# jaak-s/libfastsparse

Measured on AMD Instinct MI355X. Metric: fp64 CSR SpMV effective GB/s (% HBM3E peak), higher is better.
Workload: dtype f64

## Files before the change

libfastsparse_amd/csrc/fs_kernels_twopass.hip:

```cpp
#include <stdlib.h>

#include "fs_kernel_util.h"

namespace fs {


template <int U, bool NTLD, bool NTST, int BC>
__device__ __forceinline__ void expand_share(double *__restrict__ xband, int ncol, int B, const unsigned *__restrict__ band_ptr,
                                             const uint16_t *__restrict__ lcol, const unsigned *__restrict__ gdst,
                                             const double *__restrict__ x, int xs, double *__restrict__ prod, unsigned g0,
                                             unsigned g1)
{
  const int t = threadIdx.x;
  if (g0 >= g1) return;
  int b;
  {
    int lo = 0, hi = B - 1;
    while (lo < hi) {
      const int mid = lo + ((hi - lo + 1) >> 1);
      if (band_ptr[mid] <= g0) lo = mid; else hi = mid - 1;
    }
    b = lo;
  }
  for (unsigned g = g0; g < g1; ++b) {
    const unsigned gb = band_ptr[b + 1] < g1 ? band_ptr[b + 1] : g1;
    if (gb <= g) continue;
    const int c0 = b * BC;
    const int w = (ncol - c0 < BC) ? ncol - c0 : BC;
    __syncthreads();
    {
      double r[BC / kBinBlock];
#pragma unroll
      for (int j = 0; j < BC / kBinBlock; ++j) {
        const int i = j * kBinBlock + t;
        r[j] = __builtin_nontemporal_load(x + (int64_t)(c0 + (i < w ? i : w - 1)) * xs);
      }
#pragma unroll
      for (int j = 0; j < BC / kBinBlock; ++j) {
        const int i = j * kBinBlock + t;
        xband[i] = (i < w) ? r[j] : 0.0;
      }
      if (t < 8) xband[BC + t] = 0.0;
    }
    __syncthreads();
    const int64_t e0 = (int64_t)g * kBinGroup, e1 = (int64_t)gb * kBinGroup;
    constexpr int64_t kRound = 2 * U * kBinBlock;
    int64_t o = e0 + 2 * t;
    for (; o - 2 * t + kRound <= e1; o += kRound) {
      unsigned a[U], d[U];
#pragma unroll
      for (int k = 0; k < U; ++k) {
        const int64_t e = o + (int64_t)k * 2 * kBinBlock;
        a[k] = stream_load<NTLD>((const unsigned *)(lcol + e));
        d[k] = stream_load<NTLD>(gdst + (e >> kBinGroupLog));
      }
      __builtin_amdgcn_sched_barrier(0);
#pragma unroll
      for (int k = 0; k < U; ++k) {
        const int64_t e = o + (int64_t)k * 2 * kBinBlock;
        const v2d p = {xband[a[k] & 0xffffu], xband[a[k] >> 16]};
        stream_store<NTST>(p, (v2d *)(prod + (int64_t)d[k] * kBinGroup + (e & (kBinGroup - 1))));
      }
    }
    for (; o < e1; o += 2 * kBinBlock) {
      const unsigned a = stream_load<NTLD>((const unsigned *)(lcol + o));
      const unsigned d = stream_load<NTLD>(gdst + (o >> kBinGroupLog));
      const v2d p = {xband[a & 0xffffu], xband[a >> 16]};
      stream_store<NTST>(p, (v2d *)(prod + (int64_t)d * kBinGroup + (o & (kBinGroup - 1))));
    }
    g = gb;
  }
}

template <int U, bool NTLD, bool NTST, int BC = kBinCols>
__global__ __launch_bounds__(kBinBlock) void spmv_expand_kernel(
    int ncol, int B, const unsigned *__restrict__ band_ptr, const uint16_t *__restrict__ lcol,
    const unsigned *__restrict__ gdst, const double *__restrict__ x, int xs, double *__restrict__ prod, unsigned gbeg,
    unsigned gend)
{
  __shared__ double xband[BC + 8];
  const uint64_t groups = gend - gbeg;
  const unsigned g0 = gbeg + (unsigned)(groups * blockIdx.x / gridDim.x), g1 = gbeg + (unsigned)(groups * (blockIdx.x + 1) / gridDim.x);
  expand_share<U, NTLD, NTST, BC>(xband, ncol, B, band_ptr, lcol, gdst, x, xs, prod, g0, g1);
}

static_assert(kBinGroupLog == 4, "the one-byte row ids (row_ids, line_ids, rows8_decode_kernel) decode groups of 16 entries: two lanes of 8, eight lanes of 2, four words of 4");
template <bool NTLD, bool L8>
__device__ __forceinline__ v4u row_ids_load(const uint16_t *__restrict__ lrow, const uint8_t *__restrict__ lrow8,
                                            const uint16_t *__restrict__ gbase, int64_t e)
{
  if (!L8) return stream_load<NTLD>((const v4u *)(lrow + e));
  typedef unsigned v2u __attribute__((ext_vector_type(2)));
  const v2u d = stream_load<NTLD>((const v2u *)(lrow8 + e));
  return v4u{d.x, d.y, (unsigned)gbase[e >> kBinGroupLog], (unsigned)(e >> 3) & 1u};
}

template <bool L8>
__device__ __forceinline__ v4u row_ids(v4u raw)
{
  if (!L8) return raw;
  const unsigned dx = raw.x, dy = raw.y;
  const unsigned s0 = dx & 0xffu, s1 = s0 + ((dx >> 8) & 0xffu), s2 = s1 + ((dx >> 16) & 0xffu), s3 = s2 + (dx >> 24);
  const unsigned s4 = s3 + (dy & 0xffu), s5 = s4 + ((dy >> 8) & 0xffu), s6 = s5 + ((dy >> 16) & 0xffu), s7 = s6 + (dy >> 24);
  const unsigned below = (unsigned)__builtin_amdgcn_update_dpp(0, (int)s7, 0x111 , 0xf, 0xf, false);
  const unsigned off = raw.z + (raw.w ? below : 0u);
  return v4u{(off + s0) | ((off + s1) << 16), (off + s2) | ((off + s3) << 16), (off + s4) | ((off + s5) << 16), (off + s6) | ((off + s7) << 16)};
}

template <bool L8>
__device__ __forceinline__ unsigned line_ids_load(const uint16_t *__restrict__ lrow, const uint8_t *__restrict__ lrow8,
                                                  const uint16_t *__restrict__ gbase, int64_t e)
{
  if (!L8) return *(const unsigned *)(lrow + e);
  return (unsigned)*(const uint16_t *)(lrow8 + e) | ((unsigned)gbase[e >> kBinGroupLog] << 16);
}

template <bool L8>
__device__ __forceinline__ unsigned line_ids(unsigned raw)
{
  if (!L8) return raw;
  const unsigned d0 = raw & 0xffu, own = d0 + ((raw >> 8) & 0xffu), l = threadIdx.x & 7u;
  unsigned s = own, u;
  u = (unsigned)__builtin_amdgcn_update_dpp(0, (int)s, 0x111 , 0xf, 0xf, false); s += l >= 1 ? u : 0u;
  u = (unsigned)__builtin_amdgcn_update_dpp(0, (int)s, 0x112 , 0xf, 0xf, false); s += l >= 2 ? u : 0u;
  u = (unsigned)__builtin_amdgcn_update_dpp(0, (int)s, 0x114 , 0xf, 0xf, false); s += l >= 4 ? u : 0u;
  const unsigned off = (raw >> 16) + s - own;
  return (off + d0) | ((off + own) << 16);
}

template <bool VALUED, bool NTLD, bool L8 = false>
__device__ __forceinline__ void reduce_panel(double *__restrict__ ytile, int panel, const unsigned *__restrict__ bin_ptr,
                                             const int *__restrict__ panel_row, const uint16_t *__restrict__ lrow,
                                             const double *__restrict__ vals, const double *__restrict__ prod, double *__restrict__ y,
                                             int ys, const uint8_t *__restrict__ lrow8 = nullptr,
                                             const uint16_t *__restrict__ gbase = nullptr)
{
  const int t = threadIdx.x;
  const int r0 = panel_row[panel], nr = panel_row[panel + 1] - r0;
  for (int i = t; i < nr; i += kBinBlock) ytile[i] = 0.0;
  __syncthreads();
  const int64_t e0 = (int64_t)bin_ptr[panel] * kBinGroup, e1 = (int64_t)bin_ptr[panel + 1] * kBinGroup;
#define FS_ADD(idx, val) __hip_atomic_fetch_add(&ytile[idx], val, __ATOMIC_RELAXED, __HIP_MEMORY_SCOPE_WORKGROUP)
#define FS_ADD2(A, P) FS_ADD((A) & 0xffffu, (P).x); FS_ADD((A) >> 16, (P).y);
  constexpr int64_t kStep = 8 * kBinBlock, kRound = 2 * kStep;
  const int wave0 = (t >> 6) * 512, lane0 = wave0 + 2 * (t & 63);
  int64_t eb = e0;
  for (; eb + kRound <= e1; eb += kRound) {
    const int64_t e = eb + lane0;
    unsigned a[2][4];
    v2d p[2][4], v[2][4];
#pragma unroll
    for (int k = 0; k < 2; ++k)
#pragma unroll
      for (int j = 0; j < 4; ++j) {
        const int64_t ek = e + k * kStep + 128 * j;
        a[k][j] = line_ids_load<L8>(lrow, lrow8, gbase, ek);
        p[k][j] = stream_load<NTLD>((const v2d *)(prod + ek));
        if (VALUED) v[k][j] = stream_load<NTLD>((const v2d *)(vals + ek));
      }
    __builtin_amdgcn_sched_barrier(0);
#pragma unroll
    for (int k = 0; k < 2; ++k)
#pragma unroll
      for (int j = 0; j < 4; ++j) {
        const unsigned r = line_ids<L8>(a[k][j]);
        if (VALUED) { p[k][j].x *= v[k][j].x; p[k][j].y *= v[k][j].y; }
        FS_ADD2(r, p[k][j])
      }
  }
  for (; eb + wave0 < e1; eb += kStep) {
    const int64_t e = eb + lane0;
    unsigned a[4];
    v2d p[4], v[4];
#pragma unroll
    for (int j = 0; j < 4; ++j) {
      const int64_t ej = e + 128 * j, ec = ej < e1 ? ej : e1 - 2;
      a[j] = line_ids_load<L8>(lrow, lrow8, gbase, ec);
      p[j] = stream_load<NTLD>((const v2d *)(prod + ec));
      if (VALUED) v[j] = stream_load<NTLD>((const v2d *)(vals + ec));
    }
#pragma unroll
    for (int j = 0; j < 4; ++j) {
      const unsigned r = line_ids<L8>(a[j]);
      if (VALUED) { p[j].x *= v[j].x; p[j].y *= v[j].y; }
      if (e + 128 * j < e1) { FS_ADD2(r, p[j]) }
    }
  }
#undef FS_ADD2
#undef FS_ADD
  __syncthreads();
  for (int i = t; i < nr; i += kBinBlock) y[(int64_t)(r0 + i) * ys] = ytile[i];
}

template <bool VALUED, bool NTLD, int RM = kBinRowsMax, bool L8 = false>
__global__ __launch_bounds__(kBinBlock) void spmv_reduce_kernel(
    const unsigned *__restrict__ bin_ptr, const int *__restrict__ panel_row, const uint16_t *__restrict__ lrow,
    const double *__restrict__ vals, const double *__restrict__ prod, double *__restrict__ y, int ys, int pbase,
    const uint8_t *__restrict__ lrow8 = nullptr, const uint16_t *__restrict__ gbase = nullptr)
{
  __shared__ double ytile[RM];
  reduce_panel<VALUED, NTLD, L8>(ytile, pbase + blockIdx.x, bin_ptr, panel_row, lrow, vals, prod, y, ys, lrow8, gbase);
}

#ifndef FS_ORDERED_DEPTH
#define FS_ORDERED_DEPTH 16
#endif
#ifndef FS_ORDERED_DEPTH_VALUED
#define FS_ORDERED_DEPTH_VALUED 10
#endif
template <bool VALUED, bool NTLD, int RM, int DEPTH, bool L8 = false>
__global__ __launch_bounds__(64) void spmv_reduce_ordered_kernel(
    const unsigned *__restrict__ bin_ptr, const int *__restrict__ panel_row, const uint16_t *__restrict__ lrow,
    const double *__restrict__ vals, const double *__restrict__ prod, double *__restrict__ y, int ys, int pbase,
    const uint8_t *__restrict__ lrow8 = nullptr, const uint16_t *__restrict__ gbase = nullptr)
{
  __shared__ __attribute__((aligned(16))) double ytile[RM];
  const int t = threadIdx.x;
  const int panel = pbase + blockIdx.x;
  const int r0 = panel_row[panel], nr = panel_row[panel + 1] - r0;
  for (int i = 2 * t; i < nr; i += 128) *reinterpret_cast<v2d *>(&ytile[i]) = v2d{0.0, 0.0};
  const int64_t e0 = (int64_t)bin_ptr[panel] * kBinGroup, e1 = (int64_t)bin_ptr[panel + 1] * kBinGroup;
#define FS_ADD(idx, val) __hip_atomic_fetch_add(&ytile[idx], val, __ATOMIC_RELAXED, __HIP_MEMORY_SCOPE_WORKGROUP)
#define FS_ADD8(A, P)                                                  \
  FS_ADD(A.x & 0xffffu, P[0].x); FS_ADD(A.x >> 16, P[0].y);            \
  FS_ADD(A.y & 0xffffu, P[1].x); FS_ADD(A.y >> 16, P[1].y);            \
  FS_ADD(A.z & 0xffffu, P[2].x); FS_ADD(A.z >> 16, P[2].y);            \
  FS_ADD(A.w & 0xffffu, P[3].x); FS_ADD(A.w >> 16, P[3].y);
  constexpr int64_t kStep = 8 * 64;
  v4u a[DEPTH];
  v2d p[DEPTH][4], v[VALUED ? DEPTH : 1][4];
  auto fetch = [&](int k, int64_t e) {
    const int64_t ec = (e + 8 <= e1) ? e : (e1 - e0 >= 8 ? e1 - 8 : e0);
    a[k] = row_ids_load<NTLD, L8>(lrow, lrow8, gbase, ec);
#pragma unroll
    for (int j = 0; j < 4; ++j) {
      p[k][j] = stream_load<NTLD>((const v2d *)(prod + ec + 2 * j));
      if (VALUED) v[k][j] = stream_load<NTLD>((const v2d *)(vals + ec + 2 * j));
    }
  };
  if (e1 > e0) {
    int64_t e = e0 + 8 * t;
#pragma unroll
    for (int k = 0; k < DEPTH; ++k) fetch(k, e + (int64_t)k * kStep);
    for (; e - 8 * t < e1; e += (int64_t)DEPTH * kStep) {
#pragma unroll
      for (int k = 0; k < DEPTH; ++k) {
        const int64_t ek = e + (int64_t)k * kStep;
        const v4u ak = row_ids<L8>(a[k]);
        v2d pk[4] = {p[k][0], p[k][1], p[k][2], p[k][3]};
        if (VALUED) {
#pragma unroll
          for (int j = 0; j < 4; ++j) { pk[j].x *= v[k][j].x; pk[j].y *= v[k][j].y; }
        }
        fetch(k, ek + (int64_t)DEPTH * kStep);
        if (ek + 8 <= e1) { FS_ADD8(ak, pk) }
      }
    }
  }
#undef FS_ADD8
#undef FS_ADD
  __syncthreads();
  for (int i = t; i < nr; i += 64) y[(int64_t)(r0 + i) * ys] = ytile[i];
}

template <bool VALUED, int BC, int NACC, bool ORDERED>
__global__ __launch_bounds__(kBinBlock) void spmv_longrows_kernel(
    int ncol, int B, int nlong, const int64_t *__restrict__ band_ptr, const unsigned *__restrict__ seg_ptr,
    const uint16_t *__restrict__ lcol, const uint16_t *__restrict__ lrow, const double *__restrict__ vals,
    const double *__restrict__ x, int xs, double *__restrict__ ylong, double *__restrict__ ypart)
{
  __shared__ double xband[BC + 8];
  __shared__ double acc[NACC];
  const int t = threadIdx.x, lane = t & 63, wave = t >> 6;
  for (int i = t; i < nlong; i += kBinBlock) acc[i] = 0.0;
  const int64_t pairs = band_ptr[B] >> 1;
  const int64_t e_beg = 2 * (pairs * blockIdx.x / gridDim.x), e_end = 2 * (pairs * (blockIdx.x + 1) / gridDim.x);
  if (e_beg < e_end) {
    int b;
    {
      int lo = 0, hi = B - 1;
      while (lo < hi) {
        const int mid = lo + ((hi - lo + 1) >> 1);
        if (band_ptr[mid] <= e_beg) lo = mid; else hi = mid - 1;
      }
      b = lo;
    }
    double rn[BC / kBinBlock];
    int have = -1;
    auto request = [&](int bb) {
      const int cb = bb * BC;
      const int wb = (ncol - cb < BC) ? ncol - cb : BC;
#pragma unroll
      for (int j = 0; j < BC / kBinBlock; ++j) {
        const int i = j * kBinBlock + t;
        rn[j] = __builtin_nontemporal_load(x + (int64_t)(cb + (i < wb ? i : wb - 1)) * xs);
      }
      have = bb;
    };
    auto wave_step = [&](int64_t o, bool live, int64_t oc) {
      const unsigned a = *reinterpret_cast<const unsigned *>(lcol + oc);
      const unsigned rr = *reinterpret_cast<const unsigned *>(lrow + oc);
      v2d p = {xband[a & 0xffffu], xband[a >> 16]};
      if (VALUED) { const v2d v = *reinterpret_cast<const v2d *>(vals + oc); p.x *= v.x; p.y *= v.y; }
      unsigned key = 0xffffffffu;
      double sum = 0.0;
      if (live) {
        const unsigned r0 = rr & 0xffffu, r1 = rr >> 16;
        if (r0 == r1) { key = r0; sum = p.x + p.y; }
        else { __hip_atomic_fetch_add(&acc[r0], p.x, __ATOMIC_RELAXED, __HIP_MEMORY_SCOPE_WORKGROUP); key = r1; sum = p.y; }
      }
#pragma unroll
      for (int d = 1; d < 64; d <<= 1) {
        const unsigned ku = __shfl_up(key, d);
        const double su = __shfl_up(sum, d);
        if (lane >= d && ku == key) sum += su;
      }
      const unsigned kn = __shfl_down(key, 1);
      if (live && (lane == 63 || kn != key))
        __hip_atomic_fetch_add(&acc[key], sum, __ATOMIC_RELAXED, __HIP_MEMORY_SCOPE_WORKGROUP);
      (void)o;
    };
    for (int64_t e = e_beg; e < e_end; ++b) {
      const int64_t eb = band_ptr[b + 1] < e_end ? band_ptr[b + 1] : e_end;
      if (eb <= e) continue;
      const int c0 = b * BC;
      const int w = (ncol - c0 < BC) ? ncol - c0 : BC;
      if (have != b) request(b);
      __syncthreads();
#pragma unroll
      for (int j = 0; j < BC / kBinBlock; ++j) {
        const int i = j * kBinBlock + t;
        xband[i] = (i < w) ? rn[j] : 0.0;
      }
      if (t < 8) xband[BC + t] = 0.0;
      __syncthreads();
      if (b + 1 < B && eb < e_end) request(b + 1);
      if (ORDERED) {
        const int64_t s0 = band_ptr[b] + seg_ptr[b * (kLongOwners + 1) + wave], s1 = band_ptr[b] + seg_ptr[b * (kLongOwners + 1) + wave + 1];
        const int64_t lo = s0 > e ? s0 : e, hi = s1 < eb ? s1 : eb;
        for (int64_t o0 = lo; o0 < hi; o0 += 128) {
          const int64_t o = o0 + 2 * lane;
          const bool live = o < hi;
          wave_step(o, live, live ? o : lo);
        }
      } else {
        for (int64_t o0 = e; o0 < eb; o0 += 2 * kBinBlock) {
          const int64_t o = o0 + 2 * t;
          const bool live = o < eb;
          wave_step(o, live, live ? o : e);
        }
      }
      e = eb;
    }
  }
  __syncthreads();
  if (ORDERED) {
    double *__restrict__ mine = ypart + (int64_t)blockIdx.x * nlong;
    for (int i = t; i < nlong; i += kBinBlock) mine[i] = acc[i];
  } else {
    for (int i = t; i < nlong; i += kBinBlock) {
      const double v = acc[i];
      if (v != 0.0) unsafeAtomicAdd(ylong + i, v);
    }
  }
}

__global__ __launch_bounds__(kBlock) void longrows_combine_kernel(int nlong, int nwg, const double *__restrict__ ypart, double *__restrict__ ylong)
{
  const int i = blockIdx.x * kBlock + threadIdx.x;
  if (i >= nlong) return;
  double acc = 0.0;
  for (int w = 0; w < nwg; ++w) acc += ypart[(int64_t)w * nlong + i];
  ylong[i] = acc;
}

__global__ __launch_bounds__(kBlock) void longrows_scatter_kernel(int nlong, const int *__restrict__ row, const double *__restrict__ ylong,
                                                                 double *__restrict__ y, int ys, int row0, int row1)
{
  const int i = blockIdx.x * kBlock + threadIdx.x;
  if (i >= nlong) return;
  const int r = row[i];
  if (r >= row0 && r < row1) y[(int64_t)r * ys] = 0.0 + ylong[i];
}

static int launch_longrows(const DeviceCsr &A, const LongRows &L, const double *x, int xs, hipStream_t s)
{
  const bool ordered = reproducible_now();
  if (!ordered || L.n == 0 || L.nwg == 0)
    if (int rc = launch_zero(L.ylong, sizeof(double) * (size_t)L.nlong, s)) return rc;
  if (L.n == 0 || L.nwg == 0) return FS_OK;
#define FS_LONG(V, BC, NA, ORD)                                                                                              \
  hipLaunchKernelGGL((spmv_longrows_kernel<V, BC, NA, ORD>), dim3(L.nwg), dim3(kBinBlock), 0, s, A.ncol, L.B, L.nlong, L.band_ptr, \
                     L.seg_ptr, L.lcol, L.lrow, L.vals, x, xs, L.ylong, L.ypart)
#define FS_LONG2(V, BC, NA) do { if (ordered) FS_LONG(V, BC, NA, true); else FS_LONG(V, BC, NA, false); } while (0)
  if (L.bcols == kLongBandB) { if (A.has_vals()) FS_LONG2(true, kLongBandB, kLongRowsB); else FS_LONG2(false, kLongBandB, kLongRowsB); }
  else                       { if (A.has_vals()) FS_LONG2(true, kLongBandA, kLongRowsA); else FS_LONG2(false, kLongBandA, kLongRowsA); }
#undef FS_LONG2
#undef FS_LONG
  FS_HIP(hipGetLastError());
  if (ordered) {
    hipLaunchKernelGGL(longrows_combine_kernel, dim3((unsigned)((L.nlong + kBlock - 1) / kBlock)), dim3(kBlock), 0, s, L.nlong, L.nwg, L.ypart,
                       L.ylong);
    FS_HIP(hipGetLastError());
  }
  return FS_OK;
}


template <int K, int U>
__global__ __launch_bounds__(kBinBlock) void spmm_expand_kernel(
    int ncol, int B, const unsigned *__restrict__ band_ptr, const uint16_t *__restrict__ lcol,
    const unsigned *__restrict__ gdst, const double *__restrict__ X, int xs, double *__restrict__ prod)
{
  constexpr int BC = kBinCols / K;
  constexpr int GE = kBinGroup / K;
  constexpr int LP = K / 2;
  constexpr int EPS = kBinBlock / LP;
  __shared__ __attribute__((aligned(16))) double xband[kBinCols + 8];
  const int t = threadIdx.x;
  const int le = t / LP, h = t % LP;
  const uint64_t groups = band_ptr[B];
  const unsigned g0 = (unsigned)(groups * blockIdx.x / gridDim.x), g1 = (unsigned)(groups * (blockIdx.x + 1) / gridDim.x);
  if (g0 >= g1) return;
  int b;
  {
    int lo = 0, hi = B - 1;
    while (lo < hi) {
      const int mid = lo + ((hi - lo + 1) >> 1);
      if (band_ptr[mid] <= g0) lo = mid; else hi = mid - 1;
    }
    b = lo;
  }
  for (unsigned g = g0; g < g1; ++b) {
    const unsigned gb = band_ptr[b + 1] < g1 ? band_ptr[b + 1] : g1;
    if (gb <= g) continue;
    const int c0 = b * BC;
    const int w = (ncol - c0 < BC) ? ncol - c0 : BC;
    __syncthreads();
    {
      double r[kBinCols / kBinBlock];
#pragma unroll
      for (int j = 0; j < kBinCols / kBinBlock; ++j) {
        const int f = j * kBinBlock + t, i = f / K, q = f % K;
        r[j] = __builtin_nontemporal_load(X + (int64_t)(c0 + (i < w ? i : w - 1)) * xs + q);
      }
#pragma unroll
      for (int j = 0; j < kBinCols / kBinBlock; ++j) {
        const int f = j * kBinBlock + t;
        xband[f] = (f / K < w) ? r[j] : 0.0;
      }
      if (t < 8) xband[kBinCols + t] = 0.0;
    }
    __syncthreads();
    const int64_t e0 = (int64_t)g * GE, e1 = (int64_t)gb * GE;
    constexpr int64_t kRound = (int64_t)U * EPS;
    int64_t o = e0 + le;
    for (; o - le + kRound <= e1; o += kRound) {
      unsigned a[U], d[U];
#pragma unroll
      for (int k = 0; k < U; ++k) {
        const int64_t e = o + (int64_t)k * EPS;
        a[k] = lcol[e];
        d[k] = gdst[e / GE];
      }
      __builtin_amdgcn_sched_barrier(0);
#pragma unroll
      for (int k = 0; k < U; ++k) {
        const int64_t e = o + (int64_t)k * EPS;
        const v2d p = *reinterpret_cast<const v2d *>(&xband[a[k] * K + 2 * h]);
        __builtin_nontemporal_store(p, (v2d *)(prod + ((int64_t)d[k] * GE + (e % GE)) * K + 2 * h));
      }
    }
    for (; o < e1; o += EPS) {
      const unsigned a = lcol[o];
      const unsigned d = gdst[o / GE];
      const v2d p = *reinterpret_cast<const v2d *>(&xband[a * K + 2 * h]);
      __builtin_nontemporal_store(p, (v2d *)(prod + ((int64_t)d * GE + (o % GE)) * K + 2 * h));
    }
    g = gb;
  }
}

template <bool VALUED, int K>
__global__ __launch_bounds__(kBinBlock) void spmm_reduce_kernel(
    const unsigned *__restrict__ bin_ptr_all, const int *__restrict__ panel_row_all, const uint16_t *__restrict__ lrow,
    const double *__restrict__ vals, const double *__restrict__ prod, double *__restrict__ Y, int ys, int pbase)
{
  const unsigned *__restrict__ bin_ptr = bin_ptr_all + pbase;
  const int *__restrict__ panel_row = panel_row_all + pbase;
  constexpr int GE = kBinGroup / K;
  constexpr int EPL = 8 / K;
  __shared__ double ytile[kBinRowsMax];
  const int t = threadIdx.x;
  const int r0 = panel_row[blockIdx.x], nr = panel_row[blockIdx.x + 1] - r0;
  for (int i = t; i < nr * K; i += kBinBlock) ytile[i] = 0.0;
  __syncthreads();
  const int64_t e0 = (int64_t)bin_ptr[blockIdx.x] * GE, e1 = (int64_t)bin_ptr[blockIdx.x + 1] * GE;
  typedef uint16_t rows_t __attribute__((ext_vector_type(EPL)));
  typedef double vals_t __attribute__((ext_vector_type(EPL)));
#define FS_ADD(idx, val) __hip_atomic_fetch_add(&ytile[idx], val, __ATOMIC_RELAXED, __HIP_MEMORY_SCOPE_WORKGROUP)
  auto add8 = [&](const rows_t a, const v2d (&p)[4], const vals_t v) {
#pragma unroll
    for (int q = 0; q < EPL; ++q) {
      const int base = (int)a[q] * K;
#pragma unroll
      for (int j = 0; j < K; j += 2) {
        v2d t2 = p[(q * K + j) / 2];
        if (VALUED) { t2.x *= v[q]; t2.y *= v[q]; }
        FS_ADD(base + j, t2.x);
        FS_ADD(base + j + 1, t2.y);
      }
    }
  };
  constexpr int64_t kStep = (int64_t)EPL * kBinBlock;
  constexpr int64_t kRound = 2 * kStep;
  int64_t e = e0 + (int64_t)EPL * t;
  for (; e - EPL * t + kRound <= e1; e += kRound) {
    rows_t a[2];
    v2d p[2][4];
    vals_t v[2] = {};
#pragma unroll
    for (int k = 0; k < 2; ++k) {
      const int64_t ek = e + k * kStep;
      a[k] = *reinterpret_cast<const rows_t *>(lrow + ek);
      if (VALUED) v[k] = *reinterpret_cast<const vals_t *>(vals + ek);
#pragma unroll
      for (int j = 0; j < 4; ++j) p[k][j] = *reinterpret_cast<const v2d *>(prod + ek * K + 2 * j);
    }
    __builtin_amdgcn_sched_barrier(0);
    add8(a[0], p[0], v[0]);
    add8(a[1], p[1], v[1]);
  }
  for (; e < e1; e += kStep) {
    const rows_t a = *reinterpret_cast<const rows_t *>(lrow + e);
    vals_t v = {};
    if (VALUED) v = *reinterpret_cast<const vals_t *>(vals + e);
    v2d p[4];
#pragma unroll
    for (int j = 0; j < 4; ++j) p[j] = *reinterpret_cast<const v2d *>(prod + e * K + 2 * j);
    add8(a, p, v);
  }
#undef FS_ADD
  __syncthreads();
  for (int i = t; i < nr * K; i += kBinBlock) Y[(int64_t)(r0 + i / K) * ys + (i % K)] = ytile[i];
}

template <bool VALUED, int K, int DEPTH>
__global__ __launch_bounds__(64) void spmm_reduce_ordered_kernel(
    const unsigned *__restrict__ bin_ptr_all, const int *__restrict__ panel_row_all, const uint16_t *__restrict__ lrow,
    const double *__restrict__ vals, const double *__restrict__ prod, double *__restrict__ Y, int ys, int pbase)
{
  const unsigned *__restrict__ bin_ptr = bin_ptr_all + pbase;
  const int *__restrict__ panel_row = panel_row_all + pbase;
  constexpr int GE = kBinGroup / K;
  constexpr int EPL = 8 / K;
  __shared__ double ytile[kBinRowsMax];
  const int t = threadIdx.x;
  const int r0 = panel_row[blockIdx.x], nr = panel_row[blockIdx.x + 1] - r0;
  for (int i = t; i < nr * K; i += 64) ytile[i] = 0.0;
  const int64_t e0 = (int64_t)bin_ptr[blockIdx.x] * GE, e1 = (int64_t)bin_ptr[blockIdx.x + 1] * GE;
  typedef uint16_t rows_t __attribute__((ext_vector_type(EPL)));
  typedef double vals_t __attribute__((ext_vector_type(EPL)));
#define FS_ADD(idx, val) __hip_atomic_fetch_add(&ytile[idx], val, __ATOMIC_RELAXED, __HIP_MEMORY_SCOPE_WORKGROUP)
  auto add8 = [&](const rows_t a, const v2d (&p)[4], const vals_t v) {
#pragma unroll
    for (int q = 0; q < EPL; ++q) {
      const int base = (int)a[q] * K;
#pragma unroll
      for (int j = 0; j < K; j += 2) {
        v2d t2 = p[(q * K + j) / 2];
        if (VALUED) { t2.x *= v[q]; t2.y *= v[q]; }
        FS_ADD(base + j, t2.x);
        FS_ADD(base + j + 1, t2.y);
      }
    }
  };
  constexpr int64_t kStep = (int64_t)EPL * 64;
  rows_t a[DEPTH];
  v2d p[DEPTH][4];
  vals_t v[VALUED ? DEPTH : 1] = {};
  auto fetch = [&](int k, int64_t e) {
    const int64_t ec = (e + EPL <= e1) ? e : (e1 - e0 >= EPL ? e1 - EPL : e0);
    a[k] = *reinterpret_cast<const rows_t *>(lrow + ec);
    if (VALUED) v[k] = *reinterpret_cast<const vals_t *>(vals + ec);
#pragma unroll
    for (int j = 0; j < 4; ++j) p[k][j] = *reinterpret_cast<const v2d *>(prod + ec * K + 2 * j);
  };
  if (e1 > e0) {
    int64_t e = e0 + (int64_t)EPL * t;
#pragma unroll
    for (int k = 0; k < DEPTH; ++k) fetch(k, e + (int64_t)k * kStep);
    for (; e - EPL * t < e1; e += (int64_t)DEPTH * kStep) {
#pragma unroll
      for (int k = 0; k < DEPTH; ++k) {
        const int64_t ek = e + (int64_t)k * kStep;
        const rows_t ak = a[k];
        const v2d pk[4] = {p[k][0], p[k][1], p[k][2], p[k][3]};
        const vals_t vk = v[VALUED ? k : 0];
        fetch(k, ek + (int64_t)DEPTH * kStep);
        if (ek + EPL <= e1) add8(ak, pk, vk);
      }
    }
  }
#undef FS_ADD
  __syncthreads();
  for (int i = t; i < nr * K; i += 64) Y[(int64_t)(r0 + i / K) * ys + (i % K)] = ytile[i];
}

template <int K>
__global__ __launch_bounds__(kBlock) void tiled_combine_k_kernel(int nrow, const int *__restrict__ vfirst,
                                                                const double *__restrict__ yv, double *__restrict__ Y, int ys,
                                                                int row0 = 0)
{
  const int64_t i = (int64_t)row0 * K + (int64_t)blockIdx.x * kBlock + threadIdx.x;
  const int64_t r = i / K;
  const int j = (int)(i % K);
  if (r >= nrow) return;
  const int a = vfirst[r], b = vfirst[r + 1];
  double acc = yv[(int64_t)a * K + j];
  for (int v = a + 1; v < b; ++v) acc += yv[(int64_t)v * K + j];
  Y[r * ys + j] = acc;
}

__global__ void rows8_decode_kernel(int64_t groups, const uint8_t *__restrict__ lrow8, const uint16_t *__restrict__ gbase,
                                    uint16_t *__restrict__ lrow)
{
  const int64_t g = (int64_t)blockIdx.x * blockDim.x + threadIdx.x;
  if (g >= groups) return;
  const v4u d = *(const v4u *)(lrow8 + g * kBinGroup);
  unsigned r = gbase[g];
  unsigned out[kBinGroup / 2];
#pragma unroll
  for (int j = 0; j < kBinGroup; j += 2) {
    const unsigned w = j < 4 ? d.x : j < 8 ? d.y : j < 12 ? d.z : d.w;
    const unsigned a = r + ((w >> (8 * (j & 3))) & 0xffu), b = a + ((w >> (8 * ((j + 1) & 3))) & 0xffu);
    out[j / 2] = a | (b << 16);
    r = b;
  }
#pragma unroll
  for (int j = 0; j < kBinGroup / 8; ++j)
    *(v4u *)(lrow + g * kBinGroup + 8 * j) = v4u{out[4 * j], out[4 * j + 1], out[4 * j + 2], out[4 * j + 3]};
}

static void ensure_two_byte_ids(BinnedCsr &N, hipStream_t s)
{
  if (N.lrow || !N.lrow8 || N.lrow_tried) return;
  hipStreamCaptureStatus cap = hipStreamCaptureStatusNone;
  if (hipStreamIsCapturing(s, &cap) != hipSuccess) { (void)hipGetLastError(); return; }
  if (cap != hipStreamCaptureStatusNone) return;
  N.lrow_tried = true;
  uint16_t *p = nullptr;
  if (hipMalloc(&p, sizeof(uint16_t) * (size_t)N.n) != hipSuccess) { (void)hipGetLastError(); return; }
  const int64_t groups = N.n >> kBinGroupLog;
  if (groups > 0) hipLaunchKernelGGL(rows8_decode_kernel, dim3((unsigned)((groups + 255) / 256)), dim3(256), 0, s, groups, N.lrow8, N.gbase, p);
  if (hipGetLastError() != hipSuccess || hipStreamSynchronize(s) != hipSuccess) { (void)hipGetLastError(); (void)hipFree(p); return; }
  N.lrow = p;
}

static void launch_reduce(const BinnedCsr &N, double *out, int os, int p0, int p1, int flags, hipStream_t s)
{
#define FS_REDUCE(V, NT, RM, L8)                                                                                                \
  hipLaunchKernelGGL((spmv_reduce_kernel<V, NT, RM, L8>), dim3(p1 - p0), dim3(kBinBlock), 0, s, N.bin_ptr, N.panel_row, N.lrow, \
                     N.vals, N.prod, out, os, p0, N.lrow8, N.gbase)
#define FS_REDUCE2(RM, L8)                                                                       \
  do {                                                                                           \
    if (N.vals) { if (flags & 256) FS_REDUCE(true, false, RM, L8); else FS_REDUCE(true, true, RM, L8); }   \
    else        { if (flags & 256) FS_REDUCE(false, false, RM, L8); else FS_REDUCE(false, true, RM, L8); } \
  } while (0)
  if (N.bcols == kBinColsBig) FS_REDUCE2(kBinRowsBig, false);
  else if (N.lrow8)           FS_REDUCE2(kBinRowsMax, true);
  else                        FS_REDUCE2(kBinRowsMax, false);
#undef FS_REDUCE2
#undef FS_REDUCE
}

int launch_spmv_binned(const DeviceCsr &A, double *y, const double *x, hipStream_t s, int xs, int ys, int p0, int p1, int row0,
                       int row1)
{
  const BinnedCsr &N = *A.binned;
  double *out = N.split ? N.yv : y;
  const int os = N.split ? 1 : ys;
  const bool part = p1 >= 0;
  if (!part) { p0 = 0; p1 = N.P; row0 = 0; row1 = A.nrow; }
  const int nwg1 = (options().bin_wgs > 0 && options().bin_wgs < N.nwg1) ? options().bin_wgs : N.nwg1;
  if (nwg1 > 0 && p0 == 0) {
    const int flags = options().bin_flags;
#define FS_EXPAND4(U)                                                                                       \
  do {                                                                                                      \
    if (flags & 16) { if (flags & 8) FS_EXPAND(U, true, false);  else FS_EXPAND(U, true, true); }           \
    else            { if (flags & 8) FS_EXPAND(U, false, false); else FS_EXPAND(U, false, true); }          \
  } while (0)
#define FS_EXPAND(U, NL, NS)                                                                                      \
  hipLaunchKernelGGL((spmv_expand_kernel<U, NL, NS>), dim3(nwg1), dim3(kBinBlock), 0, s, A.ncol, N.B, N.band_ptr, \
                     N.lcol, N.gdst, x, xs, N.prod, 0u, (unsigned)(N.n >> kBinGroupLog))
    if (N.bcols == kBinColsBig)
      hipLaunchKernelGGL((spmv_expand_kernel<4, false, true, kBinColsBig>), dim3(nwg1), dim3(kBinBlock), 0, s, A.ncol, N.B,
                         N.band_ptr, N.lcol, N.gdst, x, xs, N.prod, 0u, (unsigned)(N.n >> kBinGroupLog));
    else if ((flags & 3) == 1) FS_EXPAND4(8);
    else if ((flags & 3) == 2) FS_EXPAND4(2);
    else                       FS_EXPAND4(4);
#undef FS_EXPAND4
#undef FS_EXPAND
    FS_HIP(hipGetLastError());
  }
  if (N.lr && p0 == 0)
    if (int rc = launch_longrows(A, *N.lr, x, xs, s)) return rc;
  if (p1 > p0) {
    const bool ordered = reproducible_now() || (options().bin_flags & 32);
    if (ordered && N.lrow8 && !N.lrow) ensure_two_byte_ids(*A.binned, s);
#define FS_ORDERED(RM, L8)                                                                                                     \
  do {                                                                                                                         \
    if (N.vals)                                                                                                                \
      hipLaunchKernelGGL((spmv_reduce_ordered_kernel<true, false, RM, FS_ORDERED_DEPTH_VALUED, L8>), dim3(p1 - p0), dim3(64), 0, s, \
                         N.bin_ptr, N.panel_row, N.lrow, N.vals, N.prod, out, os, p0, N.lrow8, N.gbase);                       \
    else                                                                                                                       \
      hipLaunchKernelGGL((spmv_reduce_ordered_kernel<false, false, RM, FS_ORDERED_DEPTH, L8>), dim3(p1 - p0), dim3(64), 0, s,  \
                         N.bin_ptr, N.panel_row, N.lrow, N.vals, N.prod, out, os, p0, N.lrow8, N.gbase);                       \
  } while (0)
    if (N.bcols == kBinColsBig && ordered)  FS_ORDERED(kBinRowsBig, false);
    else if (ordered && N.lrow8 && !N.lrow) FS_ORDERED(kBinRowsMax, true);
    else if (ordered)                       FS_ORDERED(kBinRowsMax, false);
    else
      launch_reduce(N, out, os, p0, p1, options().bin_flags, s);
#undef FS_ORDERED
    FS_HIP(hipGetLastError());
  }
  if (N.split && row1 > row0) {
    if (int rc = launch_tiled_combine(row1, N.vfirst, N.yv, y, ys, row0, s)) return rc;
  }
  if (N.lr && row1 > row0) {
    hipLaunchKernelGGL(longrows_scatter_kernel, dim3((unsigned)((N.lr->nlong + kBlock - 1) / kBlock)), dim3(kBlock), 0, s, N.lr->nlong,
                       N.lr->row, N.lr->ylong, y, ys, row0, row1);
    FS_HIP(hipGetLastError());
  }
  return FS_OK;
}

int launch_expand_groups(const DeviceCsr &A, const double *x, unsigned g0, unsigned g1, int wgs, hipStream_t s)
{
  const BinnedCsr &N = *A.binned;
  if (g1 <= g0 || wgs <= 0) return FS_OK;
#define FS_XH(BC)                                                                                                         \
  hipLaunchKernelGGL((spmv_expand_kernel<4, false, true, BC>), dim3(wgs), dim3(kBinBlock), 0, s, A.ncol, N.B, N.band_ptr, \
                     N.lcol, N.gdst, x, 1, N.prod, g0, g1)
  if (N.bcols == kBinColsBig) FS_XH(kBinColsBig);
  else                        FS_XH(kBinCols);
#undef FS_XH
  FS_HIP(hipGetLastError());
  return FS_OK;
}

int launch_reduce_panels(const DeviceCsr &A, double *y, int p0, int p1, hipStream_t s)
{
  const BinnedCsr &N = *A.binned;
  if (p1 <= p0) return FS_OK;
  launch_reduce(N, y, 1, p0, p1, 0, s);
  FS_HIP(hipGetLastError());
  return FS_OK;
}

int launch_spmm_binned(const DeviceCsr &A, const BinnedCsr &N, double *Y, const double *X, hipStream_t s, int xs, int ys, int p0,
                       int p1, int row0, int row1)
{
  const int K = N.kw;
  double *out = N.split ? N.yv : Y;
  const int os = N.split ? K : ys;
  if (p1 < 0) { p0 = 0; p1 = N.P; row0 = 0; row1 = A.nrow; }
  const int nwg1 = (p0 != 0) ? 0 : ((options().bin_wgs > 0 && options().bin_wgs < N.nwg1) ? options().bin_wgs : N.nwg1);
#define FS_XP(KK)                                                                                                  \
  hipLaunchKernelGGL((spmm_expand_kernel<KK, 4>), dim3(nwg1), dim3(kBinBlock), 0, s, A.ncol, N.B, N.band_ptr, N.lcol, \
                     N.gdst, X, xs, N.prod)
  if (nwg1 > 0) {
    if (K == 2) FS_XP(2); else FS_XP(4);
    FS_HIP(hipGetLastError());
  }
#undef FS_XP
  if (p1 > p0) {
    const bool ordered = reproducible_now() || (options().bin_flags & 32);
#define FS_RP(V, KK)                                                                                                            \
  do {                                                                                                                          \
    if (ordered)                                                                                                                \
      hipLaunchKernelGGL((spmm_reduce_ordered_kernel<V, KK, (V && KK == 2) ? 12 : FS_ORDERED_DEPTH>), dim3(p1 - p0), dim3(64), 0, s, N.bin_ptr, \
                         N.panel_row, N.lrow, N.vals, N.prod, out, os, p0);                                                     \
    else                                                                                                                        \
      hipLaunchKernelGGL((spmm_reduce_kernel<V, KK>), dim3(p1 - p0), dim3(kBinBlock), 0, s, N.bin_ptr, N.panel_row, N.lrow,     \
                         N.vals, N.prod, out, os, p0);                                                                          \
  } while (0)
    if (K == 2) { if (N.vals) FS_RP(true, 2); else FS_RP(false, 2); }
    else        { if (N.vals) FS_RP(true, 4); else FS_RP(false, 4); }
#undef FS_RP
    FS_HIP(hipGetLastError());
  }
  if (N.split && row1 > row0) {
    const unsigned grid = (unsigned)(((int64_t)(row1 - row0) * K + kBlock - 1) / kBlock);
    if (K == 2)
      hipLaunchKernelGGL(tiled_combine_k_kernel<2>, dim3(grid), dim3(kBlock), 0, s, row1, N.vfirst, N.yv, Y, ys, row0);
    else
      hipLaunchKernelGGL(tiled_combine_k_kernel<4>, dim3(grid), dim3(kBlock), 0, s, row1, N.vfirst, N.yv, Y, ys, row0);
    FS_HIP(hipGetLastError());
  }
  return FS_OK;
}

}
```

Before: 2679.

## Add helper prefetch waves to ordered SpMV/SpMM reduce kernels

Ordered reduce kernels gain H extra wavefronts per workgroup, 3 by default. These helpers can walk ahead of the main wave, touching prod, vals and row-id lines to warm the cache. Progress is coordinated through an LDS position counter with sleep-based throttling. The prefetch itself is compiled out by default because FS_ORDERED_WINDOW is 0, so the default effect is a 4-wave block whose extra waves only share the final y writeback. This risks wasting occupancy on idle waves, and the ordered path runs only in reproducible mode or when bin_flags has bit 32 set.

```diff
diff --git a/libfastsparse_amd/csrc/fs_kernels_twopass.hip b/libfastsparse_amd/csrc/fs_kernels_twopass.hip
--- a/libfastsparse_amd/csrc/fs_kernels_twopass.hip
+++ b/libfastsparse_amd/csrc/fs_kernels_twopass.hip
@@ -208,59 +208,140 @@
 #ifndef FS_ORDERED_DEPTH_VALUED
 #define FS_ORDERED_DEPTH_VALUED 10
 #endif
-template <bool VALUED, bool NTLD, int RM, int DEPTH, bool L8 = false>
-__global__ __launch_bounds__(64) void spmv_reduce_ordered_kernel(
+#ifndef FS_ORDERED_HELPERS
+#define FS_ORDERED_HELPERS 3
+#endif
+#ifndef FS_ORDERED_WINDOW
+#define FS_ORDERED_WINDOW 0
+#endif
+constexpr bool kOrderedPrefetch = FS_ORDERED_WINDOW > 0;
+constexpr int kOrderedChunk = 64;
+constexpr int kOrderedRing = 4;
+constexpr int kOrderedNaps = 64;
+
+__device__ __forceinline__ void ordered_publish(unsigned *pos, unsigned groups)
+{
+  __hip_atomic_store(pos, groups, __ATOMIC_RELAXED, __HIP_MEMORY_SCOPE_WORKGROUP);
+}
+
+template <bool VALUED, int K, bool L8, int H>
+__device__ __forceinline__ void ordered_helper_loop(int h, int lane, unsigned g0, unsigned g1, int64_t lead, unsigned *pos,
+                                                    const uint16_t *__restrict__ lrow, const double *__restrict__ vals,
+                                                    const double *__restrict__ prod, const uint8_t *__restrict__ lrow8,
+                                                    const uint16_t *__restrict__ gbase)
+{
+  constexpr int GE = kBinGroup / K;
+  const int64_t ng = (int64_t)g1 - (int64_t)g0;
+  if (ng <= 0) return;
+  unsigned r[kOrderedRing][4] = {};
+  auto sink = [&](int k) {
+#pragma unroll
+    for (int j = 0; j < 4; ++j) asm volatile("" ::"v"(r[k][j]));
+  };
+  constexpr int64_t stride = (int64_t)H * kOrderedChunk;
+  int64_t c = (int64_t)h * kOrderedChunk;
+  while (c < ng) {
+#pragma unroll
+    for (int k = 0; k < kOrderedRing; ++k) {
+      if (c >= ng) break;
+      int64_t asked = 0;
+      for (int naps = 0;; ++naps) {
+        asked = (int64_t)__builtin_amdgcn_readfirstlane(__hip_atomic_load(pos, __ATOMIC_RELAXED, __HIP_MEMORY_SCOPE_WORKGROUP)) + lead;
+        if (c <= asked + FS_ORDERED_WINDOW || naps >= kOrderedNaps) break;
+        __builtin_amdgcn_s_sleep(16);
+      }
+      if (c + kOrderedChunk <= asked) {
+        c += ((asked - c - kOrderedChunk) / stride + 1) * stride;
+        if (c >= ng) break;
+      }
+      const int64_t gl = c + lane < ng ? c + lane : ng - 1;
+      const int64_t g = (int64_t)g0 + gl;
+      sink(k);
+      r[k][0] = *reinterpret_cast<const unsigned *>(prod + g * kBinGroup);
+      if (VALUED) r[k][1] = *reinterpret_cast<const unsigned *>(vals + g * GE);
+      if (L8) {
+        r[k][2] = *reinterpret_cast<const unsigned *>(lrow8 + g * GE);
+        r[k][3] = gbase[g];
+      } else {
+        r[k][2] = *reinterpret_cast<const unsigned *>(lrow + g * GE);
+      }
+      c += stride;
+    }
+  }
+#pragma unroll
+  for (int k = 0; k < kOrderedRing; ++k) sink(k);
+}
+
+template <bool VALUED, bool NTLD, int RM, int DEPTH, bool L8 = false, int H = 0>
+__global__ __launch_bounds__(64 * (1 + H)) void spmv_reduce_ordered_kernel(
     const unsigned *__restrict__ bin_ptr, const int *__restrict__ panel_row, const uint16_t *__restrict__ lrow,
     const double *__restrict__ vals, const double *__restrict__ prod, double *__restrict__ y, int ys, int pbase,
     const uint8_t *__restrict__ lrow8 = nullptr, const uint16_t *__restrict__ gbase = nullptr)
 {
   __shared__ __attribute__((aligned(16))) double ytile[RM];
+  __shared__ unsigned pos[1];
   const int t = threadIdx.x;
   const int panel = pbase + blockIdx.x;
   const int r0 = panel_row[panel], nr = panel_row[panel + 1] - r0;
-  for (int i = 2 * t; i < nr; i += 128) *reinterpret_cast<v2d *>(&ytile[i]) = v2d{0.0, 0.0};
-  const int64_t e0 = (int64_t)bin_ptr[panel] * kBinGroup, e1 = (int64_t)bin_ptr[panel + 1] * kBinGroup;
+  const int wave = H > 0 ? __builtin_amdgcn_readfirstlane(t >> 6) : 0;
+  if (H > 0 && kOrderedPrefetch) {
+    if (t == 0) ordered_publish(pos, 0u);
+    __syncthreads();
+    if (wave > 0)
+      ordered_helper_loop<VALUED, 1, L8, (H > 0 ? H : 1)>(wave - 1, t & 63, bin_ptr[panel], bin_ptr[panel + 1], DEPTH * (512 / kBinGroup), pos,
+                                                          lrow, vals, prod, lrow8, gbase);
+  }
+  if (wave == 0) {
+    for (int i = 2 * t; i < nr; i += 128) *reinterpret_cast<v2d *>(&ytile[i]) = v2d{0.0, 0.0};
+    const int64_t e0 = (int64_t)bin_ptr[panel] * kBinGroup, e1 = (int64_t)bin_ptr[panel + 1] * kBinGroup;
 #define FS_ADD(idx, val) __hip_atomic_fetch_add(&ytile[idx], val, __ATOMIC_RELAXED, __HIP_MEMORY_SCOPE_WORKGROUP)
 #define FS_ADD8(A, P)                                                  \
-  FS_ADD(A.x & 0xffffu, P[0].x); FS_ADD(A.x >> 16, P[0].y);            \
-  FS_ADD(A.y & 0xffffu, P[1].x); FS_ADD(A.y >> 16, P[1].y);            \
-  FS_ADD(A.z & 0xffffu, P[2].x); FS_ADD(A.z >> 16, P[2].y);            \
-  FS_ADD(A.w & 0xffffu, P[3].x); FS_ADD(A.w >> 16, P[3].y);
-  constexpr int64_t kStep = 8 * 64;
-  v4u a[DEPTH];
-  v2d p[DEPTH][4], v[VALUED ? DEPTH : 1][4];
-  auto fetch = [&](int k, int64_t e) {
-    const int64_t ec = (e + 8 <= e1) ? e : (e1 - e0 >= 8 ? e1 - 8 : e0);
-    a[k] = row_ids_load<NTLD, L8>(lrow, lrow8, gbase, ec);
-#pragma unroll
-    for (int j = 0; j < 4; ++j) {
-      p[k][j] = stream_load<NTLD>((const v2d *)(prod + ec + 2 * j));
-      if (VALUED) v[k][j] = stream_load<NTLD>((const v2d *)(vals + ec + 2 * j));
-    }
-  };
-  if (e1 > e0) {
-    int64_t e = e0 + 8 * t;
-#pragma unroll
-    for (int k = 0; k < DEPTH; ++k) fetch(k, e + (int64_t)k * kStep);
-    for (; e - 8 * t < e1; e += (int64_t)DEPTH * kStep) {
-#pragma unroll
-      for (int k = 0; k < DEPTH; ++k) {
-        const int64_t ek = e + (int64_t)k * kStep;
-        const v4u ak = row_ids<L8>(a[k]);
-        v2d pk[4] = {p[k][0], p[k][1], p[k][2], p[k][3]};
-        if (VALUED) {
-#pragma unroll
-          for (int j = 0; j < 4; ++j) { pk[j].x *= v[k][j].x; pk[j].y *= v[k][j].y; }
+    FS_ADD(A.x & 0xffffu, P[0].x); FS_ADD(A.x >> 16, P[0].y);            \
+    FS_ADD(A.y & 0xffffu, P[1].x); FS_ADD(A.y >> 16, P[1].y);            \
+    FS_ADD(A.z & 0xffffu, P[2].x); FS_ADD(A.z >> 16, P[2].y);            \
+    FS_ADD(A.w & 0xffffu, P[3].x); FS_ADD(A.w >> 16, P[3].y);
+    constexpr int64_t kStep = 8 * 64;
+    v4u a[DEPTH];
+    v2d p[DEPTH][4], v[VALUED ? DEPTH : 1][4];
+    auto fetch = [&](int k, int64_t e) {
+      const int64_t ec = (e + 8 <= e1) ? e : (e1 - e0 >= 8 ? e1 - 8 : e0);
+      a[k] = row_ids_load<NTLD, L8>(lrow, lrow8, gbase, ec);
+#pragma unroll
+      for (int j = 0; j < 4; ++j) {
+        p[k][j] = stream_load<NTLD>((const v2d *)(prod + ec + 2 * j));
+        if (VALUED) v[k][j] = stream_load<NTLD>((const v2d *)(vals + ec + 2 * j));
+      }
+    };
+    if (e1 > e0) {
+      int64_t e = e0 + 8 * t;
+#pragma unroll
+      for (int k = 0; k < DEPTH; ++k) fetch(k, e + (int64_t)k * kStep);
+      for (; e - 8 * t < e1; e += (int64_t)DEPTH * kStep) {
+        if (H > 0 && kOrderedPrefetch && t == 0) ordered_publish(pos, (unsigned)((e - e0) >> kBinGroupLog));
+#pragma unroll
+        for (int k = 0; k < DEPTH; ++k) {
+          const int64_t ek = e + (int64_t)k * kStep;
+          const v4u ak = row_ids<L8>(a[k]);
+          v2d pk[4] = {p[k][0], p[k][1], p[k][2], p[k][3]};
+          if (VALUED) {
+#pragma unroll
+            for (int j = 0; j < 4; ++j) { pk[j].x *= v[k][j].x; pk[j].y *= v[k][j].y; }
+          }
+          fetch(k, ek + (int64_t)DEPTH * kStep);
+          if (ek + 8 <= e1) { FS_ADD8(ak, pk) }
         }
-        fetch(k, ek + (int64_t)DEPTH * kStep);
-        if (ek + 8 <= e1) { FS_ADD8(ak, pk) }
-      }
-    }
-  }
+      }
+    }
 #undef FS_ADD8
 #undef FS_ADD
+  }
   __syncthreads();
-  for (int i = t; i < nr; i += 64) y[(int64_t)(r0 + i) * ys] = ytile[i];
+  if (H == 0) {
+    for (int i = t; i < nr; i += 64) y[(int64_t)(r0 + i) * ys] = ytile[i];
+  } else {
+#pragma unroll 8
+    for (int i = t; i < nr; i += 64 * (1 + H)) y[(int64_t)(r0 + i) * ys] = ytile[i];
+  }
 }
 
 template <bool VALUED, int BC, int NACC, bool ORDERED>
@@ -545,8 +626,8 @@
   for (int i = t; i < nr * K; i += kBinBlock) Y[(int64_t)(r0 + i / K) * ys + (i % K)] = ytile[i];
 }
 
-template <bool VALUED, int K, int DEPTH>
-__global__ __launch_bounds__(64) void spmm_reduce_ordered_kernel(
+template <bool VALUED, int K, int DEPTH, int H = 0>
+__global__ __launch_bounds__(64 * (1 + H)) void spmm_reduce_ordered_kernel(
     const unsigned *__restrict__ bin_ptr_all, const int *__restrict__ panel_row_all, const uint16_t *__restrict__ lrow,
     const double *__restrict__ vals, const double *__restrict__ prod, double *__restrict__ Y, int ys, int pbase)
 {
@@ -555,56 +636,73 @@
   constexpr int GE = kBinGroup / K;
   constexpr int EPL = 8 / K;
   __shared__ double ytile[kBinRowsMax];
+  __shared__ unsigned pos[1];
   const int t = threadIdx.x;
   const int r0 = panel_row[blockIdx.x], nr = panel_row[blockIdx.x + 1] - r0;
-  for (int i = t; i < nr * K; i += 64) ytile[i] = 0.0;
-  const int64_t e0 = (int64_t)bin_ptr[blockIdx.x] * GE, e1 = (int64_t)bin_ptr[blockIdx.x + 1] * GE;
-  typedef uint16_t rows_t __attribute__((ext_vector_type(EPL)));
-  typedef double vals_t __attribute__((ext_vector_type(EPL)));
+  const int wave = H > 0 ? __builtin_amdgcn_readfirstlane(t >> 6) : 0;
+  if (H > 0 && kOrderedPrefetch) {
+    if (t == 0) ordered_publish(pos, 0u);
+    __syncthreads();
+    if (wave > 0)
+      ordered_helper_loop<VALUED, K, false, (H > 0 ? H : 1)>(wave - 1, t & 63, bin_ptr[blockIdx.x], bin_ptr[blockIdx.x + 1], DEPTH * (64 * EPL / GE),
+                                                             pos, lrow, vals, prod, nullptr, nullptr);
+  }
+  if (wave == 0) {
+    for (int i = t; i < nr * K; i += 64) ytile[i] = 0.0;
+    const int64_t e0 = (int64_t)bin_ptr[blockIdx.x] * GE, e1 = (int64_t)bin_ptr[blockIdx.x + 1] * GE;
+    typedef uint16_t rows_t __attribute__((ext_vector_type(EPL)));
+    typedef double vals_t __attribute__((ext_vector_type(EPL)));
 #define FS_ADD(idx, val) __hip_atomic_fetch_add(&ytile[idx], val, __ATOMIC_RELAXED, __HIP_MEMORY_SCOPE_WORKGROUP)
-  auto add8 = [&](const rows_t a, const v2d (&p)[4], const vals_t v) {
-#pragma unroll
-    for (int q = 0; q < EPL; ++q) {
-      const int base = (int)a[q] * K;
-#pragma unroll
-      for (int j = 0; j < K; j += 2) {
-        v2d t2 = p[(q * K + j) / 2];
-        if (VALUED) { t2.x *= v[q]; t2.y *= v[q]; }
-        FS_ADD(base + j, t2.x);
-        FS_ADD(base + j + 1, t2.y);
-      }
-    }
-  };
-  constexpr int64_t kStep = (int64_t)EPL * 64;
-  rows_t a[DEPTH];
-  v2d p[DEPTH][4];
-  vals_t v[VALUED ? DEPTH : 1] = {};
-  auto fetch = [&](int k, int64_t e) {
-    const int64_t ec = (e + EPL <= e1) ? e : (e1 - e0 >= EPL ? e1 - EPL : e0);
-    a[k] = *reinterpret_cast<const rows_t *>(lrow + ec);
-    if (VALUED) v[k] = *reinterpret_cast<const vals_t *>(vals + ec);
-#pragma unroll
-    for (int j = 0; j < 4; ++j) p[k][j] = *reinterpret_cast<const v2d *>(prod + ec * K + 2 * j);
-  };
-  if (e1 > e0) {
-    int64_t e = e0 + (int64_t)EPL * t;
-#pragma unroll
-    for (int k = 0; k < DEPTH; ++k) fetch(k, e + (int64_t)k * kStep);
-    for (; e - EPL * t < e1; e += (int64_t)DEPTH * kStep) {
-#pragma unroll
-      for (int k = 0; k < DEPTH; ++k) {
-        const int64_t ek = e + (int64_t)k * kStep;
-        const rows_t ak = a[k];
-        const v2d pk[4] = {p[k][0], p[k][1], p[k][2], p[k][3]};
-        const vals_t vk = v[VALUED ? k : 0];
-        fetch(k, ek + (int64_t)DEPTH * kStep);
-        if (ek + EPL <= e1) add8(ak, pk, vk);
-      }
-    }
-  }
+    auto add8 = [&](const rows_t a, const v2d (&p)[4], const vals_t v) {
+#pragma unroll
+      for (int q = 0; q < EPL; ++q) {
+        const int base = (int)a[q] * K;
+#pragma unroll
+        for (int j = 0; j < K; j += 2) {
+          v2d t2 = p[(q * K + j) / 2];
+          if (VALUED) { t2.x *= v[q]; t2.y *= v[q]; }
+          FS_ADD(base + j, t2.x);
+          FS_ADD(base + j + 1, t2.y);
+        }
+      }
+    };
+    constexpr int64_t kStep = (int64_t)EPL * 64;
+    rows_t a[DEPTH];
+    v2d p[DEPTH][4];
+    vals_t v[VALUED ? DEPTH : 1] = {};
+    auto fetch = [&](int k, int64_t e) {
+      const int64_t ec = (e + EPL <= e1) ? e : (e1 - e0 >= EPL ? e1 - EPL : e0);
+      a[k] = *reinterpret_cast<const rows_t *>(lrow + ec);
+      if (VALUED) v[k] = *reinterpret_cast<const vals_t *>(vals + ec);
+#pragma unroll
+      for (int j = 0; j < 4; ++j) p[k][j] = *reinterpret_cast<const v2d *>(prod + ec * K + 2 * j);
+    };
+    if (e1 > e0) {
+      int64_t e = e0 + (int64_t)EPL * t;
+#pragma unroll
+      for (int k = 0; k < DEPTH; ++k) fetch(k, e + (int64_t)k * kStep);
+      for (; e - EPL * t < e1; e += (int64_t)DEPTH * kStep) {
+        if (H > 0 && kOrderedPrefetch && t == 0) ordered_publish(pos, (unsigned)((e - e0) / GE));
+#pragma unroll
+        for (int k = 0; k < DEPTH; ++k) {
+          const int64_t ek = e + (int64_t)k * kStep;
+          const rows_t ak = a[k];
+          const v2d pk[4] = {p[k][0], p[k][1], p[k][2], p[k][3]};
+          const vals_t vk = v[VALUED ? k : 0];
+          fetch(k, ek + (int64_t)DEPTH * kStep);
+          if (ek + EPL <= e1) add8(ak, pk, vk);
+        }
+      }
+    }
 #undef FS_ADD
+  }
   __syncthreads();
-  for (int i = t; i < nr * K; i += 64) Y[(int64_t)(r0 + i / K) * ys + (i % K)] = ytile[i];
+  if (H == 0) {
+    for (int i = t; i < nr * K; i += 64) Y[(int64_t)(r0 + i / K) * ys + (i % K)] = ytile[i];
+  } else {
+#pragma unroll 8
+    for (int i = t; i < nr * K; i += 64 * (1 + H)) Y[(int64_t)(r0 + i / K) * ys + (i % K)] = ytile[i];
+  }
 }
 
 template <int K>
@@ -708,14 +806,18 @@
   if (p1 > p0) {
     const bool ordered = reproducible_now() || (options().bin_flags & 32);
     if (ordered && N.lrow8 && !N.lrow) ensure_two_byte_ids(*A.binned, s);
-#define FS_ORDERED(RM, L8)                                                                                                     \
-  do {                                                                                                                         \
-    if (N.vals)                                                                                                                \
-      hipLaunchKernelGGL((spmv_reduce_ordered_kernel<true, false, RM, FS_ORDERED_DEPTH_VALUED, L8>), dim3(p1 - p0), dim3(64), 0, s, \
-                         N.bin_ptr, N.panel_row, N.lrow, N.vals, N.prod, out, os, p0, N.lrow8, N.gbase);                       \
-    else                                                                                                                       \
-      hipLaunchKernelGGL((spmv_reduce_ordered_kernel<false, false, RM, FS_ORDERED_DEPTH, L8>), dim3(p1 - p0), dim3(64), 0, s,  \
-                         N.bin_ptr, N.panel_row, N.lrow, N.vals, N.prod, out, os, p0, N.lrow8, N.gbase);                       \
+#define FS_ORDERED1(V, D, RM, L8, HW)                                                                                          \
+  hipLaunchKernelGGL((spmv_reduce_ordered_kernel<V, false, RM, D, L8, HW>), dim3(p1 - p0), dim3(64 * (1 + HW)), 0, s, N.bin_ptr, \
+                     N.panel_row, N.lrow, N.vals, N.prod, out, os, p0, N.lrow8, N.gbase)
+#define FS_ORDERED(RM, L8)                                                                                 \
+  do {                                                                                                     \
+    if (options().bin_flags & 512) {                                                                       \
+      if (N.vals) FS_ORDERED1(true, FS_ORDERED_DEPTH_VALUED, RM, L8, 0);                                   \
+      else        FS_ORDERED1(false, FS_ORDERED_DEPTH, RM, L8, 0);                                         \
+    } else {                                                                                               \
+      if (N.vals) FS_ORDERED1(true, FS_ORDERED_DEPTH_VALUED, RM, L8, FS_ORDERED_HELPERS);                  \
+      else        FS_ORDERED1(false, FS_ORDERED_DEPTH, RM, L8, FS_ORDERED_HELPERS);                        \
+    }                                                                                                      \
   } while (0)
     if (N.bcols == kBinColsBig && ordered)  FS_ORDERED(kBinRowsBig, false);
     else if (ordered && N.lrow8 && !N.lrow) FS_ORDERED(kBinRowsMax, true);
@@ -723,6 +825,7 @@
     else
       launch_reduce(N, out, os, p0, p1, options().bin_flags, s);
 #undef FS_ORDERED
+#undef FS_ORDERED1
     FS_HIP(hipGetLastError());
   }
   if (N.split && row1 > row0) {
@@ -777,11 +880,15 @@
 #undef FS_XP
   if (p1 > p0) {
     const bool ordered = reproducible_now() || (options().bin_flags & 32);
+#define FS_RPO(V, KK, HW)                                                                                                       \
+  hipLaunchKernelGGL((spmm_reduce_ordered_kernel<V, KK, (V && KK == 2) ? 12 : FS_ORDERED_DEPTH, HW>), dim3(p1 - p0),              \
+                     dim3(64 * (1 + HW)), 0, s, N.bin_ptr, N.panel_row, N.lrow, N.vals, N.prod, out, os, p0)
 #define FS_RP(V, KK)                                                                                                            \
   do {                                                                                                                          \
-    if (ordered)                                                                                                                \
-      hipLaunchKernelGGL((spmm_reduce_ordered_kernel<V, KK, (V && KK == 2) ? 12 : FS_ORDERED_DEPTH>), dim3(p1 - p0), dim3(64), 0, s, N.bin_ptr, \
-                         N.panel_row, N.lrow, N.vals, N.prod, out, os, p0);                                                     \
+    if (ordered && (options().bin_flags & 512))                                                \
+      FS_RPO(V, KK, 0);                                                                                                         \
+    else if (ordered)                                                                                                           \
+      FS_RPO(V, KK, FS_ORDERED_HELPERS);                                                                                        \
     else                                                                                                                        \
       hipLaunchKernelGGL((spmm_reduce_kernel<V, KK>), dim3(p1 - p0), dim3(kBinBlock), 0, s, N.bin_ptr, N.panel_row, N.lrow,     \
                          N.vals, N.prod, out, os, p0);                                                                          \
@@ -789,6 +896,7 @@
     if (K == 2) { if (N.vals) FS_RP(true, 2); else FS_RP(false, 2); }
     else        { if (N.vals) FS_RP(true, 4); else FS_RP(false, 4); }
 #undef FS_RP
+#undef FS_RPO
     FS_HIP(hipGetLastError());
   }
   if (N.split && row1 > row0) {
```

Result: slower. 2637 (-1.6%).
